# bayesian-optimization/BayesianOptimization

Measured on AMD Instinct MI355X. Metric: acquisition candidates/sec (suggest step: GP fit at fixed theta + posterior + acquisition + arg-best), higher is better.
Workload: dtype f64

## Files before the change

### bayesianoptimization_amd/_lib.py

```python
from __future__ import annotations

import ctypes as C
import os

import numpy as np

_HERE = os.path.dirname(os.path.abspath(__file__))
LIB_PATH = os.path.join(_HERE, "libgpbo.so")
DEBUG_LIB_PATH = os.path.join(_HERE, "libgpbo_dbg.so")

GPBO_OK = 0
ERR_INVALID, ERR_HIP, ERR_NOT_PD, ERR_STATE, ERR_UNSUPPORTED, ERR_COMM, ERR_PEER = -1, -2, -3, -4, -5, -6, -7
MAX_MODELS = 8
MAX_DIM = 64
MAX_SEEDS = 64
ABI_VERSION = 2

_c_double_p = C.POINTER(C.c_double)
_c_int64_p = C.POINTER(C.c_int64)
_c_int_p = C.POINTER(C.c_int)

SIGNATURES = {
    "gpbo_abi_version": (C.c_int, []),
    "gpbo_device_count": (C.c_int, [C.POINTER(C.c_int)]),
# ... 64 lines not shown
    "gpbo_group_fit_append": (C.c_int, [C.c_void_p, C.c_int, _c_double_p, C.c_int64, C.c_int, _c_double_p, C.c_int64,
                                        C.POINTER(C.c_int)]),
    "gpbo_group_lml_batch": (C.c_int, [C.c_void_p, C.c_int, _c_double_p, _c_double_p, C.c_int64, C.c_int, C.c_int, _c_double_p,
                                       C.c_int, C.c_double, C.c_int, _c_double_p, _c_double_p, C.POINTER(C.c_int),
                                       C.POINTER(C.c_int)]),
    "gpbo_group_set_candidates": (C.c_int, [C.c_void_p, _c_double_p, C.c_int64, C.c_int]),
    "gpbo_group_generate_candidates_mt19937": (C.c_int, [C.c_void_p, C.c_int64, C.c_int, _c_double_p, _c_double_p,
                                                         C.POINTER(C.c_uint32), C.POINTER(C.c_int)]),
    "gpbo_group_shard": (C.c_int, [C.c_void_p, C.c_int, _c_int64_p, _c_int64_p]),
    "gpbo_group_posterior": (C.c_int, [C.c_void_p, C.c_int, C.c_double, C.c_double, _c_double_p, _c_double_p]),
    "gpbo_group_acq_argbest": (C.c_int, [C.c_void_p, C.c_int, C.c_double, C.c_double, C.c_int, _c_double_p,
                                         _c_double_p, C.c_int, _c_int64_p, _c_double_p, _c_int64_p, _c_double_p,
                                         _c_double_p]),
    "gpbo_group_get_candidate_rows": (C.c_int, [C.c_void_p, _c_int64_p, C.c_int, _c_double_p]),
    "gpbo_polish_seeds": (C.c_int, [C.c_void_p, C.c_int, C.c_double, C.c_double, C.c_int, _c_double_p, _c_double_p, _c_double_p,
                                    _c_double_p, _c_double_p, C.c_int, C.c_int, _c_double_p, _c_double_p, C.c_int, _c_double_p,
                                    _c_double_p, C.POINTER(C.c_int), C.POINTER(C.c_int), C.POINTER(C.c_int), C.POINTER(C.c_int)]),
    "gpbo_evolve_mixed": (C.c_int, [C.c_void_p, C.c_int, C.c_double, C.c_double, C.c_double, C.c_double, C.c_int, _c_int_p,
                                    _c_int_p, _c_int_p, _c_double_p, _c_double_p, _c_double_p, C.c_int, C.c_int, C.c_int,
                                    C.POINTER(C.c_uint32), _c_int_p, _c_double_p, _c_double_p, _c_int_p, _c_int_p, _c_int_p]),
    "gpbo_mfma_f64_peak": (C.c_int, [C.c_void_p, C.c_int, _c_double_p]),
    "gpbo_mfma_f64_probe": (C.c_int, [C.c_void_p, C.c_int, C.c_int, C.c_int, _c_double_p]),
    "gpbo_hbm_copy_peak": (C.c_int, [C.c_void_p, C.c_int64, _c_double_p]),
}

DEBUG_SIGNATURES = {
    "gpbo_debug_minimize_box": (C.c_int, [C.c_void_p, C.c_void_p, _c_double_p, C.c_int, C.c_int, _c_double_p, _c_double_p, C.c_int,
                                          _c_double_p, _c_double_p, C.POINTER(C.c_int), C.POINTER(C.c_int), C.POINTER(C.c_int),
                                          C.POINTER(C.c_int)]),
    "gpbo_group_debug_create": (C.c_int, [C.c_int, C.POINTER(C.c_void_p)]),
    "gpbo_group_debug_run": (C.c_int, [C.c_void_p, C.c_int, C.c_int, C.c_int, C.c_int]),
    "gpbo_debug_cholesky": (C.c_int, [C.c_void_p, _c_double_p, C.c_int64, C.c_int, C.c_int, _c_double_p, _c_double_p,
                                      C.POINTER(C.c_int64), C.POINTER(C.c_double), C.POINTER(C.c_int)]),
    "gpbo_debug_latency_probe": (C.c_int, [C.c_void_p, C.POINTER(C.c_int64), C.c_int]),
    "gpbo_debug_select": (C.c_int, [C.c_void_p, C.c_void_p, C.c_int64, C.c_int, C.c_int, C.c_int, C.POINTER(C.c_int64), C.c_void_p,
                                    C.POINTER(C.c_int64), C.POINTER(C.c_float)]),
    "gpbo_debug_gemm": (C.c_int, [C.c_void_p, C.c_int, C.c_int, C.c_int, C.c_double, _c_double_p, _c_double_p,
                                  C.c_int, C.c_double, _c_double_p]),
    "gpbo_debug_gemm_bench": (C.c_int, [C.c_void_p, C.c_int, C.c_int, C.c_int, C.c_int, C.c_int, C.c_int, C.c_int,
                                        _c_double_p]),
    "gpbo_hybrid_probe": (C.c_int, [C.c_void_p, C.c_int, C.c_int, _c_double_p]),
    "gpbo_debug_fail_next_acq": (C.c_int, [C.c_void_p]),
    "gpbo_debug_evolve_eval": (C.c_int, [C.c_void_p, C.c_int, C.c_double, C.c_double, C.c_double, C.c_double, C.c_int, _c_int_p,
                                         _c_int_p, _c_int_p, _c_double_p, C.c_int, C.c_int, _c_double_p]),
    "gpbo_debug_evolve_walk": (C.c_int, [C.c_void_p, _c_double_p, _c_double_p, C.c_double, C.c_double, C.c_int, _c_int_p, _c_int_p,
                                         _c_int_p, _c_double_p, _c_double_p, _c_double_p, C.c_int, C.c_int, C.c_int, C.c_int,
                                         C.POINTER(C.c_uint32), _c_int_p, _c_double_p, _c_double_p, _c_int_p, _c_int_p, _c_int_p,
                                         _c_int_p]),
    "gpbo_debug_polish_eval": (C.c_int, [C.c_void_p, C.c_int, C.c_double, C.c_double, C.c_double, C.c_double, _c_double_p, C.c_int, C.c_int,
                                         C.c_int, _c_double_p]),
    "gpbo_debug_i8_pack_w": (C.c_int, [C.c_void_p, _c_double_p, C.c_int64, C.c_int64, C.c_void_p, _c_int_p, _c_double_p]),
    "gpbo_debug_i8_kstar_digits": (C.c_int, [C.c_void_p, C.c_int64, C.c_int64, C.c_int64, C.c_void_p, _c_double_p, _c_double_p]),
    "gpbo_debug_i8_gemm": (C.c_int, [C.c_void_p, C.c_void_p, _c_double_p, C.c_void_p, C.c_int64, C.c_int64, _c_double_p]),
}

_lib = None
_debug_lib = None


class GpboError(RuntimeError):
    """HIP / state / communicator failure reported by libgpbo."""


def _bind(path: str, signatures: dict):
    lib = C.CDLL(path)
    for name, (res, args) in signatures.items():
        fn = getattr(lib, name)
        fn.restype = res
        fn.argtypes = args
    if lib.gpbo_abi_version() != ABI_VERSION:
        raise ImportError(f"libgpbo ABI {lib.gpbo_abi_version()} != expected {ABI_VERSION}; rebuild")
    return lib


def load_library(path: str | None = None):
    global _lib
    if _lib is not None and path is None:
        return _lib
    explicit = path is not None
    path = path or LIB_PATH
    if not os.path.exists(path) and not explicit:
        try:
            from .build import build
            build(verbose=False)
        except Exception as e:
            raise ImportError(f"{path} not found and building it failed ({e}). There is no CPU fallback.") from e
    if not os.path.exists(path):
        raise ImportError(
            f"{path} not found: the HIP extension has not been built. Run "
            "`python -m bayesianoptimization_amd.build` (needs hipcc). There is no CPU fallback.")
    lib = _bind(path, SIGNATURES)
    if not explicit:
        _lib = lib
    return lib


def load_debug_library():
    global _debug_lib
    if _debug_lib is None:
        if not os.path.exists(DEBUG_LIB_PATH):
            try:
                from .build import build_debug
                build_debug(verbose=False)
            except Exception as e:
                raise ImportError(f"{DEBUG_LIB_PATH} not found and building it failed ({e})") from e
        _debug_lib = _bind(DEBUG_LIB_PATH, {**SIGNATURES, **DEBUG_SIGNATURES})
# ... 40 lines not shown
```

### bayesianoptimization_amd/csrc/i8_digits.h

```cpp
#pragma once

#include <cmath>
#include <cstdint>

#include "posterior_plan.h"

#if defined(__HIPCC__)
#define GPBO_HD __host__ __device__
#else
#define GPBO_HD
#endif

namespace gpbo {

static_assert((int64_t)I8_S * 128 * 128 * I8_NP_MAX < ((int64_t)1 << 31), "int32 level sums overflow at I8_NP_MAX");

template <int S>
GPBO_HD constexpr int64_t i8_offset() {
  int64_t o = 0;
  for (int t = 1; t < S; ++t) o = o * 256 + 128;
  return o;
}

GPBO_HD inline int64_t i8_round(double x) {
#if defined(__HIP_DEVICE_COMPILE__)
  return __double2ll_rn(x);
#else
  return (int64_t)std::nearbyint(x);
#endif
}

template <int S>
GPBO_HD inline int64_t i8_quantize(double x) {
  return i8_round(std::ldexp(x, 8 * S - 2)) + i8_offset<S>();
}

template <int S>
GPBO_HD inline uint32_t i8_digit_byte(int64_t Qo, int t) {
  return (uint32_t)((Qo >> (8 * (S - 1 - t))) & 255) ^ (t ? 128u : 0u);
}

GPBO_HD inline int i8_row_exponent(double maxabs) {
  int e = 0;
  (void)std::frexp(maxabs, &e);
  return maxabs > 0.0 ? e : 0;
}

template <int S>
GPBO_HD constexpr int64_t i8_frag_index(int64_t first_step, int64_t k, int plane, int item) {
  return ((first_step + (k >> 6)) * S + plane) * 64 + ((k >> 4) & 3) * 16 + item;
}
GPBO_HD constexpr int64_t i8_kd_block(int64_t cb, int64_t NP) { return cb * (NP / 64); }
GPBO_HD constexpr int64_t i8_wd_block(int64_t b) {
  const int64_t q = b >> 2, r = b & 3;
  return b + 2 * q * (q - 1) + r * q;
}

template <int S>
GPBO_HD inline double i8_combine(const int32_t* acc) {
  static_assert(S >= 5 && S <= 7, "groups of S - 4, 2 and 2 levels");
  double h = 0.0;
  for (int l = 0; l < S - 4; ++l) h = h * 256.0 + (double)acc[l];
  h *= 4294967296.0;
  const double m = (double)acc[S - 4] * 16777216.0 + (double)acc[S - 3] * 65536.0;
  const double lo = (double)acc[S - 2] * 256.0 + (double)acc[S - 1];
  const double s = h + m;
  const double bb = s - h;
  const double e = (h - (s - bb)) + (m - bb);
  return s + (e + lo);
}

template <int S>
GPBO_HD constexpr int i8_scale_exp(int e) {
  return e - 2 * (8 * S - 2) + 8 * (S - 1);
}

}
```

### bayesianoptimization_amd/csrc/posterior_i8.hip

```cpp
#include <algorithm>

#include "gpbo_internal.h"
#include "i8_digits.h"
#include "posterior_tile.h"

namespace gpbo {

typedef int v4i __attribute__((ext_vector_type(4)));

constexpr int I8_CANDS = 64;

__global__ __launch_bounds__(256) void wd_row_scale_kernel(const double* __restrict__ W, int* __restrict__ wexp,
                                                           double* __restrict__ wscale, int64_t N, int64_t NP) {
  const int64_t row = (int64_t)blockIdx.x * 4 + (threadIdx.x >> 6);
  const int lane = threadIdx.x & 63;
  if (row >= NP) return;
  double mx = 0.0;
  if (row < N)
    for (int64_t j = lane; j <= row; j += 64) mx = fmax(mx, fabs(W[row * NP + j]));
#pragma unroll
  for (int o = 32; o > 0; o >>= 1) mx = fmax(mx, __shfl_xor(mx, o));
  if (lane == 0) {
    const int e = i8_row_exponent(mx);
    wexp[row] = e;
// ... 199 lines not shown
  GPBO_HIP(ctx, hipSetDevice(ctx->device));
  Model m;
  m.N = N; m.NP = NP;
  auto done = [&](int code) {
    if (m.W) (void)hipFree(m.W);
    if (m.Wd) (void)hipFree(m.Wd);
    if (m.wscale) (void)hipFree(m.wscale);
    return code;
  };
  const size_t sq = (size_t)NP * NP * sizeof(double);
  if (hipMalloc((void**)&m.W, sq) != hipSuccess) return done(GPBO_ERR_HIP);
  if (hipMemcpy(m.W, W, sq, hipMemcpyHostToDevice) != hipSuccess) return done(GPBO_ERR_HIP);
  int rc = pack_wd(ctx, m);
  if (rc) return done(rc);
  if (hipStreamSynchronize(ctx->stream) != hipSuccess) return done(GPBO_ERR_HIP);
  const size_t wd_bytes = (size_t)i8_wd_block(NP / 16) * I8_S * 64 * sizeof(uint4);
  if (hipMemcpy(Wd_out, m.Wd, wd_bytes, hipMemcpyDeviceToHost) != hipSuccess) return done(GPBO_ERR_HIP);
  if (hipMemcpy(wscale_out, m.wscale, (size_t)NP * sizeof(double), hipMemcpyDeviceToHost) != hipSuccess) return done(GPBO_ERR_HIP);
  if (hipMemcpy(wexp_out, m.wscale + NP, (size_t)NP * sizeof(int), hipMemcpyDeviceToHost) != hipSuccess) return done(GPBO_ERR_HIP);
  return done(GPBO_OK);
}

int gpbo_debug_i8_gemm(gpbo_ctx* ctx, const void* Wd, const double* wscale, const void* Kd, int64_t NP, int64_t M, double* part_out) {
  if (!ctx) return GPBO_ERR_INVALID;
  if (!Wd || !wscale || !Kd || !part_out || !i8_debug_np_ok(NP) || M < I8_CANDS || M % I8_CANDS || M > (1 << 20))
    GPBO_FAIL(ctx, GPBO_ERR_INVALID, "debug_i8_gemm: bad arguments (NP a multiple of 64 in [64, 16384], M a multiple of 64)");
  GPBO_HIP(ctx, hipSetDevice(ctx->device));
  const int nchunks = (int)((NP + I8_ROWS - 1) / I8_ROWS);
  const size_t wd_bytes = (size_t)i8_wd_block(NP / 16) * I8_S * 64 * sizeof(uint4);
  const size_t kd_bytes = (size_t)M * NP * I8_S;
  const size_t part_bytes = (size_t)nchunks * M * sizeof(double);
  uint4 *dW = nullptr, *dK = nullptr;
  double *dS = nullptr, *dP = nullptr;
  auto done = [&](int code) {
    if (dW) (void)hipFree(dW);
    if (dK) (void)hipFree(dK);
    if (dS) (void)hipFree(dS);
    if (dP) (void)hipFree(dP);
    return code;
  };
  if (hipMalloc((void**)&dW, wd_bytes) != hipSuccess || hipMalloc((void**)&dK, kd_bytes) != hipSuccess ||
      hipMalloc((void**)&dS, (size_t)NP * sizeof(double)) != hipSuccess || hipMalloc((void**)&dP, part_bytes) != hipSuccess)
    return done(GPBO_ERR_HIP);
  if (hipMemcpy(dW, Wd, wd_bytes, hipMemcpyHostToDevice) != hipSuccess || hipMemcpy(dK, Kd, kd_bytes, hipMemcpyHostToDevice) != hipSuccess ||
      hipMemcpy(dS, wscale, (size_t)NP * sizeof(double), hipMemcpyHostToDevice) != hipSuccess ||
      hipMemset(dP, 0xff, part_bytes) != hipSuccess)
    return done(GPBO_ERR_HIP);
  const int rc = launch_i8_gemm(ctx, dW, dS, dK, dP, NP, M, nchunks, M, 0);
  if (rc) return done(rc);
  if (hipStreamSynchronize(ctx->stream) != hipSuccess) return done(GPBO_ERR_HIP);
  if (hipMemcpy(part_out, dP, part_bytes, hipMemcpyDeviceToHost) != hipSuccess) return done(GPBO_ERR_HIP);
  return done(GPBO_OK);
}
#endif
```

### bayesianoptimization_amd/csrc/posterior_kernel_v2.hip

```cpp
#include <type_traits>

#include "gpbo_internal.h"
#include "fit_bodies.h"
#include "i8_digits.h"
#include "posterior_tile.h"

namespace gpbo {

typedef double d4 __attribute__((ext_vector_type(4)));

constexpr int V2_CANDS = 64;
constexpr int V2_STRIDE = 64;

struct PostArgs2 {
  const double* Wp;
  const double* Xs;
  const double* alpha;
  const double* Xcs;
  double* part;
  double* mu_part;
  PostGrid g;
  const double* Kst;
  int64_t ldk;
  int64_t m0;
  int fuse_ends = 0;
  PostEnds ends = {};
};

template <int DP, int KERNEL, int GEN, int BK = POST_BK, int WAVES = 8>
__global__ __launch_bounds__(WAVES * 64, 4) void posterior_kernel_v2(PostArgs2 p) {
  static_assert(GEN == 1 || GEN == 2, "k* generated in the kernel or read from a slab");
  static_assert(BK == 16 || BK == 32, "stages of 16 or 32 train points");
  static_assert(WAVES == 8 || (WAVES == 16 && GEN == 1 && BK == 32), "the 16-wave form is the fused kernel with 32-point stages");
  constexpr int NT = WAVES * 64;
  constexpr int ROWS = WAVES * 32;
  constexpr int E = BK / WAVES;
  static_assert(GEN == 2 || E == 2 || E == 4, "the in-kernel generation computes train points in pairs: one or two pairs per thread and stage");
  constexpr int KP = BK / 8;
  extern __shared__ __attribute__((aligned(16))) double smem2[];
  double* Ks = smem2;
  double* Xl = smem2 + 2 * BK * V2_STRIDE;

  const int tid = threadIdx.x;
  const int wave = __builtin_amdgcn_readfirstlane(tid >> 6);
  const int lane = tid & 63;
  int r, ct;
  p.g.map(blockIdx.x, r, ct);
  const bool last = (r == p.g.nchunks - 1);
  const int NP = p.g.NP;
  const int k_end = min(NP, (r + 1) * ROWS);
  const int n_stages = k_end / BK;

  if constexpr (GEN != 2) {
    if (p.fuse_ends) {
      for (int e = tid; e < V2_CANDS * DP; e += NT) {
        const int cnd = e / DP, t = e - cnd * DP;
        const int64_t row = (int64_t)ct * V2_CANDS + cnd;
        double v = 0.0;
        if (row < p.ends.M && t < p.ends.d) v = p.ends.Xc[row * p.ends.d + t] / p.ends.ls[t];
        Xl[t * V2_CANDS + cnd] = v;
      }
    } else {
// ... 139 lines not shown
  for (; s <= last_stage; ++s) stage(s, std::integral_constant<int, 0>{});

  static_assert(2 * WAVES * V2_CANDS <= 2 * BK * V2_STRIDE, "the epilogue's exchange area aliases the stage tiles");
  double* red = Ks;
  double* mured = Ks + WAVES * V2_CANDS;
#pragma unroll
  for (int jt = 0; jt < 4; ++jt) {
    double v = 0.0;
#pragma unroll
    for (int rr = 0; rr < 4; ++rr) v = fma(acc[0][jt][rr], acc[0][jt][rr], v);
    if (!activeA) v = 0.0;
    double vb = 0.0;
#pragma unroll
    for (int rr = 0; rr < 4; ++rr) vb = fma(acc[1][jt][rr], acc[1][jt][rr], vb);
    if (activeB) v += vb;
    v += __shfl_xor(v, 16);
    v += __shfl_xor(v, 32);
    if (lane < 16) red[wave * V2_CANDS + jt * 16 + lane] = v;
  }
  mured[wave * V2_CANDS + lane] = mu_acc;
  __syncthreads();
  if (tid < V2_CANDS) {
    double v = 0.0;
#pragma unroll
    for (int w = 0; w < WAVES; ++w) v += red[w * V2_CANDS + tid];
    const int64_t m = p.m0 + (int64_t)ct * V2_CANDS + tid;
    if (GEN != 2 && p.fuse_ends) {
      double u = 0.0;
#pragma unroll
      for (int w = 0; w < WAVES; ++w) u += mured[w * V2_CANDS + tid];
      if (m < p.ends.M)
        posterior_finalize_elem(0.0 + v, 0.0 + u, p.ends.y_mean, p.ends.y_std, p.ends.mu + m, p.ends.sd + m, p.ends.negvar);
      return;
    }
    p.part[(int64_t)r * p.g.Mp + m] = v;
    if (GEN != 2 && last) {
      double u = 0.0;
#pragma unroll
      for (int w = 0; w < WAVES; ++w) u += mured[w * V2_CANDS + tid];
      p.mu_part[m] = u;
    }
  }
}

constexpr int GEN_CH = 64;
template <PostPath SLAB> struct slab_value { using type = double; };
template <> struct slab_value<PostPath::SlabF32> { using type = float; };
template <int DP, int KERNEL, PostPath SLAB>
__global__ __launch_bounds__(256) void kstar_gen_kernel(const double* __restrict__ Xs, const double* __restrict__ alpha,
                                                        const double* __restrict__ Xcs, void* __restrict__ slab,
                                                        int64_t ldk, int NP, double* __restrict__ mu_part,
                                                        int64_t Mp, int64_t m0) {
  static_assert(SLAB == PostPath::SlabF64 || SLAB == PostPath::SlabF32 || SLAB == PostPath::SlabI8, "a slab path");
  __shared__ __attribute__((aligned(16))) double xs[GEN_CH * DP];
  __shared__ double al[GEN_CH];
  const int64_t ml = (int64_t)blockIdx.x * 256 + threadIdx.x;
  const bool live = ml < ldk;
  const int k0 = blockIdx.y * POST_ROWS, k1 = min(NP, k0 + POST_ROWS);
  double xc[DP];
  {
    const double* xcp = Xcs + (m0 + (live ? ml : 0)) * DP;
#pragma unroll
    for (int t = 0; t < DP; t += 2) {
      const double2 v = *reinterpret_cast<const double2*>(xcp + t);
      xc[t] = v.x;
      xc[t + 1] = v.y;
    }
  }
  double mu = 0.0;
  auto pair = [&](int kk, double& ka, double& kb) {
    const double* xr = xs + kk * DP;
    double d2a = 0.0, d2b = 0.0;
#pragma unroll
    for (int t = 0; t < DP; ++t) {
      const double da = xc[t] - xr[t], db = xc[t] - xr[DP + t];
      d2a = fma(da, da, d2a);
      d2b = fma(db, db, d2b);
    }
    ka = gpbo_kernel_value<KERNEL>(d2a);
    kb = gpbo_kernel_value<KERNEL>(d2b);
  };
  auto mean = [&](int kk, double ka, double kb) {
    mu = fma(ka, al[kk], mu);
    mu = fma(kb, al[kk + 1], mu);
  };
  for (int kc = k0; kc < k1; kc += GEN_CH) {
    __syncthreads();
    {
      const double2* src = reinterpret_cast<const double2*>(Xs + (int64_t)kc * DP);
      double2* dst = reinterpret_cast<double2*>(xs);
      for (int e = threadIdx.x; e < GEN_CH * DP / 2; e += 256) dst[e] = src[e];
      if (threadIdx.x < GEN_CH) al[threadIdx.x] = alpha[kc + threadIdx.x];
    }
    __syncthreads();
    if (!live) continue;
    if constexpr (SLAB == PostPath::SlabI8) {
      constexpr int S = I8_S;
      uint4* Kd = static_cast<uint4*>(slab);
      const int64_t cb = i8_kd_block(ml >> 4, NP);
#pragma unroll 1
      for (int kg = 0; kg < GEN_CH; kg += 16) {
        uint32_t w[S][4] = {};
#pragma unroll
        for (int kk = kg; kk < kg + 16; kk += 2) {
          double ka, kb;
          pair(kk, ka, kb);
          mean(kk, ka, kb);
          const int64_t qa = i8_quantize<S>(ka), qb = i8_quantize<S>(kb);
          const int j = kk - kg;
#pragma unroll
          for (int t = 0; t < S; ++t) {
            w[t][j >> 2] |= (uint32_t)((qa >> (8 * (S - 1 - t))) & 255) << (8 * (j & 3));
            w[t][j >> 2] |= (uint32_t)((qb >> (8 * (S - 1 - t))) & 255) << (8 * ((j + 1) & 3));
          }
        }
        const int k = kc + kg;
        uint4* dst = Kd + i8_frag_index<S>(cb, k, 0, (int)(ml & 15));
#pragma unroll
        for (int t = 0; t < S; ++t) {
          const uint32_t x = t ? 0x80808080u : 0u;
          dst[t * 64] = make_uint4(w[t][0] ^ x, w[t][1] ^ x, w[t][2] ^ x, w[t][3] ^ x);
        }
      }
    } else {
      using T = typename slab_value<SLAB>::type;
      T* Kst = static_cast<T*>(slab);
#pragma unroll 2
      for (int kk = 0; kk < GEN_CH; kk += 2) {
        double ka, kb;
        pair(kk, ka, kb);
        const int k = kc + kk;
        Kst[(int64_t)k * ldk + ml] = (T)ka;
        Kst[(int64_t)(k + 1) * ldk + ml] = (T)kb;
        mean(kk, ka, kb);
      }
    }
  }
  if (live) mu_part[(int64_t)blockIdx.y * Mp + m0 + ml] = mu;
}

template <PostPath SLAB>
static int launch_gen(gpbo_ctx* ctx, Model& m, void* slab, int64_t ldk, int64_t Mp, int64_t m0, int nchunks) {
  return with_dp_kernel(ctx, m.DP, m.kernel, [&](auto dp, auto k) {
    kstar_gen_kernel<decltype(dp)::value, decltype(k)::value, SLAB><<<dim3((unsigned)((ldk + 255) / 256), (unsigned)nchunks), dim3(256), 0,
                                                                      ctx->stream>>>(m.Xs, m.alpha, ctx->Xcs, slab, ldk, (int)m.NP,
                                                                                     ctx->mu_part, Mp, m0);
    GPBO_HIP(ctx, hipGetLastError());
    return GPBO_OK;
  });
}

int launch_kstar_slab(gpbo_ctx* ctx, Model& m, double* Kst, int64_t ldk, int64_t Mp, int64_t m0, int nchunks) {
  return launch_gen<PostPath::SlabF64>(ctx, m, Kst, ldk, Mp, m0, nchunks);
}
int launch_kstar_slab_f32(gpbo_ctx* ctx, Model& m, float* Kst, int64_t ldk, int64_t Mp, int64_t m0, int nchunks) {
  return launch_gen<PostPath::SlabF32>(ctx, m, Kst, ldk, Mp, m0, nchunks);
}
int launch_kstar_digits(gpbo_ctx* ctx, Model& m, void* Kd, int64_t ldk, int64_t Mp, int64_t m0, int nchunks) {
  return launch_gen<PostPath::SlabI8>(ctx, m, Kd, ldk, Mp, m0, nchunks);
}

static PostArgs2 post_args(gpbo_ctx* ctx, const Model& m, int64_t Mp, int nchunks, int64_t ncands) {
  PostArgs2 a;
  a.Wp = m.Wp; a.Xs = m.Xs; a.alpha = m.alpha; a.Xcs = ctx->Xcs; a.part = ctx->part; a.mu_part = ctx->mu_part;
  a.g = {(int)m.NP, Mp, nchunks, (int)(ncands / V2_CANDS)};
  a.Kst = nullptr; a.ldk = 0; a.m0 = 0;
  return a;
}

int launch_slab_gemm_f64(gpbo_ctx* ctx, Model& m, const double* slab, int64_t ldk, int64_t m0, int64_t Mp, int part_chunks) {
  PostArgs2 a = post_args(ctx, m, Mp, part_chunks, ldk);
  a.Kst = slab; a.ldk = ldk; a.m0 = m0;
  const size_t lds = (size_t)(2 * 32 * V2_STRIDE) * sizeof(double);
  posterior_kernel_v2<4, 0, 2, 32><<<dim3((unsigned)a.g.blocks()), dim3(512), lds, ctx->stream>>>(a);
  GPBO_HIP(ctx, hipGetLastError());
  return GPBO_OK;
}

int launch_posterior_fused(gpbo_ctx* ctx, Model& m, int64_t Mp, const PostPlan& plan, const PostEnds& ends) {
  if (plan.fuse_ends && plan.part_chunks != 1) GPBO_FAIL(ctx, GPBO_ERR_STATE, "posterior: fused ends need one row chunk");
  PostArgs2 a = post_args(ctx, m, Mp, plan.part_chunks, Mp);
  const int64_t nblocks = a.g.blocks();
  if (nblocks > 0x7fffffffLL) GPBO_FAIL(ctx, GPBO_ERR_UNSUPPORTED, "posterior: grid too large; shard the candidates");
  if (plan.fuse_ends) { a.fuse_ends = 1; a.ends = ends; }
  const bool wide = plan.path == PostPath::Fused512;
  return with_dp_kernel(ctx, m.DP, m.kernel, [&](auto dp, auto k) {
    constexpr int DP = decltype(dp)::value, KERNEL = decltype(k)::value;
    if (wide) {
      const size_t lds = (size_t)(2 * 32 * V2_STRIDE + DP * V2_CANDS) * sizeof(double);
      posterior_kernel_v2<DP, KERNEL, 1, 32, 16><<<dim3((unsigned)nblocks), dim3(1024), lds, ctx->stream>>>(a);
// ... 56 lines not shown
```

### bayesianoptimization_amd/engine.py

```python
from __future__ import annotations

import contextlib
import ctypes as C
import json

import numpy as np

from . import _lib
from ._lib import dptr, iptr

RBF, MATERN25 = 0, 1
UCB, EI, POI = 0, 1, 2
F64, F32 = 0, 1

TIMING_NAMES = ("fit", "posterior_main", "posterior_finalize", "acq_argbest", "kmat", "cholesky", "trtri")


def advance_mt19937(random_state, n_words: int, lib=None):
    lib = lib or _lib.load_library()
    name, key, pos, has_gauss, cached = random_state.get_state(legacy=True)
    if name != "MT19937":
        raise TypeError("advance_mt19937 needs an MT19937 RandomState")
    n_words = int(n_words)
    avail = 624 - int(pos)
# ... 531 lines not shown
        first_nan, ms = C.c_int64(-1), C.c_float(0.0)
        self._check(self._lib.gpbo_debug_select(self._h, dptr(ys), ys.shape[0], int(k), int(variant), int(iters),
                                                idx.ctypes.data_as(C.POINTER(C.c_int64)), dptr(vals), C.byref(first_nan), C.byref(ms)))
        return idx, vals, int(first_nan.value), float(ms.value)

    def latency_probe(self, n=16):
        self._need_debug("gpbo_debug_latency_probe")
        out = np.zeros(32, dtype=np.int64)
        self._check(self._lib.gpbo_debug_latency_probe(self._h, out.ctypes.data_as(C.POINTER(C.c_int64)), int(n)))
        return out[:n]

    def debug_gemm(self, A, B, C_in=None, alpha=1.0, beta=0.0, b_trans=False):
        self._need_debug("gpbo_debug_gemm")
        A = np.ascontiguousarray(A, dtype=np.float64)
        B = np.ascontiguousarray(B, dtype=np.float64)
        m, k = A.shape
        n = B.shape[0] if b_trans else B.shape[1]
        Cm = np.zeros((m, n)) if C_in is None else np.ascontiguousarray(C_in, dtype=np.float64).copy()
        self._check(self._lib.gpbo_debug_gemm(self._h, m, n, k, float(alpha), dptr(A), dptr(B), int(b_trans),
                                              float(beta), dptr(Cm)))
        return Cm

    I8_S = 7

    @staticmethod
    def _i8_wd_bytes(NP: int) -> int:
        q = NP // 64
        return (NP // 16 + 2 * q * (q - 1)) * GpEngine.I8_S * 64 * 16

    def debug_i8_pack_w(self, W, N: int):
        self._need_debug("gpbo_debug_i8_pack_w")
        W = np.ascontiguousarray(W, dtype=np.float64)
        NP = W.shape[0]
        if W.ndim != 2 or W.shape[1] != NP or NP % 64 or not 64 <= NP <= 16384:
            raise ValueError("debug_i8_pack_w: W must be NP x NP, NP a multiple of 64 in [64, 16384]")
        Wd = np.empty(self._i8_wd_bytes(NP), dtype=np.int8)
        wexp = np.empty(NP, dtype=np.int32)
        wscale = np.empty(NP)
        self._check(self._lib.gpbo_debug_i8_pack_w(self._h, dptr(W), int(N), NP, Wd.ctypes.data_as(C.c_void_p),
                                                   wexp.ctypes.data_as(C.POINTER(C.c_int)), dptr(wscale)))
        return Wd, wexp, wscale

    def debug_i8_kstar_digits(self, NP: int, m0: int, ldk: int):
        self._need_debug("gpbo_debug_i8_kstar_digits")
        if NP % 64 or not 64 <= NP <= 16384 or ldk < 64:
            raise ValueError("debug_i8_kstar_digits: NP a multiple of 64 in [64, 16384], ldk >= 64")
        Kd = np.empty(int(ldk) * NP * self.I8_S, dtype=np.int8)
        kst = np.empty((NP, int(ldk)))
        mu_part = np.empty((2, (NP + 255) // 256, int(ldk)))
        self._check(self._lib.gpbo_debug_i8_kstar_digits(self._h, int(NP), int(m0), int(ldk), Kd.ctypes.data_as(C.c_void_p), dptr(kst),
                                                         dptr(mu_part)))
        return Kd, kst, mu_part

    def debug_i8_gemm(self, Wd, wscale, Kd, NP: int, M: int):
        self._need_debug("gpbo_debug_i8_gemm")
        Wd = np.ascontiguousarray(Wd, dtype=np.int8)
        Kd = np.ascontiguousarray(Kd, dtype=np.int8)
        wscale = np.ascontiguousarray(wscale, dtype=np.float64)
        if NP % 64 or not 64 <= NP <= 16384 or M % 64 or M < 64:
            raise ValueError("debug_i8_gemm: NP a multiple of 64 in [64, 16384], M a multiple of 64")
        if Wd.size != self._i8_wd_bytes(NP) or Kd.size != M * NP * self.I8_S or wscale.size != NP:
            raise ValueError("debug_i8_gemm: operand sizes do not match NP and M")
        part = np.empty(((NP + 127) // 128, M))
        self._check(self._lib.gpbo_debug_i8_gemm(self._h, Wd.ctypes.data_as(C.c_void_p), dptr(wscale), Kd.ctypes.data_as(C.c_void_p),
                                                 NP, M, dptr(part)))
        return part

    def gemm_bench(self, m, n, k, b_trans=True, a_trans=False, lower_only=False, iters=10) -> dict:
        self._need_debug("gpbo_debug_gemm_bench")
        out = np.zeros(2)
        self._check(self._lib.gpbo_debug_gemm_bench(self._h, int(m), int(n), int(k), int(b_trans), int(a_trans),
                                                    int(lower_only), int(iters), dptr(out)))
        return {"ms": float(out[0]), "tflops": float(out[1])}

    def mfma_f64_peak(self, iters=20000) -> float:
        out = C.c_double(0.0)
        self._check(self._lib.gpbo_mfma_f64_peak(self._h, int(iters), C.byref(out)))
        return out.value

    def mfma_f64_probe(self, iters=20000, waves_per_simd=1, mode=0) -> dict:
        out = np.zeros(4)
        self._check(self._lib.gpbo_mfma_f64_probe(self._h, int(iters), int(waves_per_simd), int(mode), dptr(out)))
        return {"tflops": out[0], "cycles_per_mfma": out[1], "shader_mhz": out[2], "ms": out[3]}

    def hybrid_probe(self, iters=2000, cfg=2) -> dict:
        self._need_debug("gpbo_hybrid_probe")
        out = np.zeros(3)
        self._check(self._lib.gpbo_hybrid_probe(self._h, int(iters), int(cfg), dptr(out)))
        return {"ms": out[0], "mfma_tflops": out[1], "valu_tflops": out[2]}

    def hbm_copy_peak(self, nbytes=1 << 30) -> float:
        out = C.c_double(0.0)
        self._check(self._lib.gpbo_hbm_copy_peak(self._h, int(nbytes), C.byref(out)))
        return out.value

    @staticmethod
    def comm_unique_id() -> bytes:
        lib = _lib.load_library()
        buf = C.create_string_buffer(128)
        rc = lib.gpbo_comm_unique_id(buf)
        if rc != _lib.GPBO_OK:
            _lib.raise_for_status(lib, None, rc)
        return buf.raw

    def comm_init(self, unique_id: bytes, world_size: int, rank: int):
        assert len(unique_id) == 128
# ... 278 lines not shown
```

### include/gpbo.h

```cpp
#ifndef GPBO_H
#define GPBO_H

#include <stdint.h>

#ifdef __cplusplus
extern "C" {
#endif

#define GPBO_ABI_VERSION 2

enum gpbo_status {
  GPBO_OK = 0,
  GPBO_ERR_INVALID = -1,
  GPBO_ERR_HIP = -2,
  GPBO_ERR_NOT_PD = -3,
  GPBO_ERR_STATE = -4,
  GPBO_ERR_UNSUPPORTED = -5,
  GPBO_ERR_COMM = -6,
  GPBO_ERR_PEER = -7
};

enum gpbo_kernel { GPBO_KERNEL_RBF = 0, GPBO_KERNEL_MATERN25 = 1 };
enum gpbo_acq { GPBO_ACQ_UCB = 0, GPBO_ACQ_EI = 1, GPBO_ACQ_POI = 2 };
enum gpbo_precision { GPBO_F64 = 0, GPBO_F32 = 1 };
// ... 107 lines not shown
                   const double* length_scale, int n_ls, double noise, int precision, int* info);
int gpbo_group_fit_append(gpbo_group* grp, int slot, const double* x_new, int64_t n_new, int d, const double* y_norm,
                          int64_t n_total, int* info);
int gpbo_group_lml_batch(gpbo_group* grp, int n_theta, const double* X, const double* y_norm, int64_t N, int d, int kernel,
                         const double* length_scales, int n_ls, double noise, int eval_gradient, double* lml, double* grad,
                         int* info, int* lane_device);
int gpbo_group_set_candidates(gpbo_group* grp, const double* Xc, int64_t M, int d);
int gpbo_group_shard(const gpbo_group* grp, int rank, int64_t* row_begin, int64_t* row_end);
int gpbo_group_generate_candidates_mt19937(gpbo_group* grp, int64_t M, int d, const double* lo, const double* hi,
                                           uint32_t* key, int* pos);
int gpbo_group_posterior(gpbo_group* grp, int slot, double y_mean, double y_std, double* mu, double* sd);
int gpbo_group_acq_argbest(gpbo_group* grp, int acq, double acq_param, double y_max, int n_constraints,
                           const double* lb, const double* ub, int k_seeds, int64_t* best_idx, double* best_val,
                           int64_t* seed_idx, double* seed_val, double* ys_out);
int gpbo_group_get_candidate_rows(gpbo_group* grp, const int64_t* idx, int n, double* out);

int gpbo_mfma_f64_peak(gpbo_ctx* ctx, int iters, double* tflops);
int gpbo_mfma_f64_probe(gpbo_ctx* ctx, int iters, int waves_per_simd, int mode, double* out);
int gpbo_hbm_copy_peak(gpbo_ctx* ctx, int64_t bytes, double* gbps);

#ifdef GPBO_DEBUG
typedef int (*gpbo_fg_callback)(const double* x, int n_live, int d, double* f, double* g, void* user);
int gpbo_debug_minimize_box(gpbo_fg_callback fg, void* user, const double* seeds, int n_seeds, int d, const double* box_lo,
                            const double* box_hi, int max_iter, double* x_out, double* f_out, int* status_out, int* n_rounds_out,
                            int* n_iter_out, int* n_eval_out);

int gpbo_debug_polish_eval(gpbo_ctx* ctx, int acq, double acq_param, double y_max, double y_mean, double y_std, const double* points,
                           int n, int d, int repeat, double* out);

int gpbo_debug_evolve_eval(gpbo_ctx* ctx, int acq, double acq_param, double y_max, double y_mean, double y_std, int n_groups,
                           const int* kind, const int* col0, const int* ncols, const double* points, int n, int D, double* out);
int gpbo_debug_evolve_walk(gpbo_ctx* ctx, const double* weights, const double* targets, double nan_below, double inf_above,
                           int n_groups, const int* kind, const int* col0, const int* ncols, const double* bounds_lo,
                           const double* bounds_hi, const double* init, int S, int D, int maxiter, int budget, unsigned* key,
                           int* pos, double* x_out, double* f_out, int* nit_out, int* nfev_out, int* success_out,
                           int* launches_out);

int gpbo_group_debug_create(int n_ranks, gpbo_group** out);
int gpbo_group_debug_run(gpbo_group* grp, int fail_rank, int fail_code, int hang_rank, int hang_ms);
int gpbo_debug_fail_next_acq(gpbo_ctx* ctx);
int gpbo_debug_cholesky(gpbo_ctx* ctx, const double* A, int64_t n, int variant, int iters, double* L_out, double* dinv_out,
                        long long* stamps_out, double* ms_out, int* info_out);
int gpbo_debug_gemm(gpbo_ctx* ctx, int m, int n, int k, double alpha, const double* A,
                    const double* B, int b_trans, double beta, double* C);
int gpbo_debug_gemm_bench(gpbo_ctx* ctx, int m, int n, int k, int b_trans, int a_trans, int lower_only, int iters,
                          double* out);
int gpbo_debug_select(gpbo_ctx* ctx, const double* ys, int64_t M, int k, int variant, int iters, int64_t* idx_out,
                      double* val_out, int64_t* first_nan_out, float* ms_out);
int gpbo_debug_latency_probe(gpbo_ctx* ctx, long long* out, int n);
int gpbo_hybrid_probe(gpbo_ctx* ctx, int iters, int cfg, double* out);
int gpbo_debug_i8_pack_w(gpbo_ctx* ctx, const double* W, int64_t N, int64_t NP, void* Wd_out, int* wexp_out, double* wscale_out);
int gpbo_debug_i8_kstar_digits(gpbo_ctx* ctx, int64_t NP, int64_t m0, int64_t ldk, void* Kd_out, double* kst_out, double* mu_part_out);
int gpbo_debug_i8_gemm(gpbo_ctx* ctx, const void* Wd, const double* wscale, const void* Kd, int64_t NP, int64_t M, double* part_out);
#endif

#ifdef __cplusplus
}
#endif
#endif
```

Before: 5.959 million.

## Double-buffer K* generation tiles and split int8 digits via byte permutes

The K* generation kernel now double-buffers the X/alpha chunk in shared memory and prefetches the next chunk into registers while computing the current one, so global loads overlap with kernel evaluation and one barrier per chunk is dropped. For the int8 slab path with small dimension, quantization into digit planes uses a magic-constant double trick plus v_perm byte shuffles on four values at once, replacing per-digit shifts and ORs. The change adds register pressure from the prefetch buffer and a second shared-memory buffer, which may lower occupancy. A debug entry point for testing the split is also added.

New measurement: 6.004 million, median of 6. No clear change (+0.8%).

```diff
diff --git a/bayesianoptimization_amd/_lib.py b/bayesianoptimization_amd/_lib.py
--- a/bayesianoptimization_amd/_lib.py
+++ b/bayesianoptimization_amd/_lib.py
@@ -140,6 +140,7 @@
     "gpbo_debug_i8_pack_w": (C.c_int, [C.c_void_p, _c_double_p, C.c_int64, C.c_int64, C.c_void_p, _c_int_p, _c_double_p]),
     "gpbo_debug_i8_kstar_digits": (C.c_int, [C.c_void_p, C.c_int64, C.c_int64, C.c_int64, C.c_void_p, _c_double_p, _c_double_p]),
     "gpbo_debug_i8_gemm": (C.c_int, [C.c_void_p, C.c_void_p, _c_double_p, C.c_void_p, C.c_int64, C.c_int64, _c_double_p]),
+    "gpbo_debug_i8_split": (C.c_int, [C.c_void_p, _c_double_p, C.c_int64, C.c_void_p]),
 }
 
 _lib = None
diff --git a/bayesianoptimization_amd/csrc/i8_digits.h b/bayesianoptimization_amd/csrc/i8_digits.h
--- a/bayesianoptimization_amd/csrc/i8_digits.h
+++ b/bayesianoptimization_amd/csrc/i8_digits.h
@@ -2,6 +2,7 @@
 
 #include <cmath>
 #include <cstdint>
+#include <cstring>
 
 #include "posterior_plan.h"
 
@@ -40,6 +41,66 @@
   return (uint32_t)((Qo >> (8 * (S - 1 - t))) & 255) ^ (t ? 128u : 0u);
 }
 
+
+GPBO_HD inline uint32_t i8_perm(uint32_t hi, uint32_t lo, uint32_t sel) {
+#if defined(__HIP_DEVICE_COMPILE__)
+  return __builtin_amdgcn_perm(hi, lo, sel);
+#else
+  const uint64_t v = ((uint64_t)hi << 32) | lo;
+  uint32_t r = 0;
+  for (int i = 0; i < 4; ++i) r |= (uint32_t)((v >> (8 * ((sel >> (8 * i)) & 7))) & 255) << (8 * i);
+  return r;
+#endif
+}
+
+GPBO_HD inline void i8_double_words(double x, uint32_t& lo, uint32_t& hi) {
+  uint64_t b;
+  std::memcpy(&b, &x, sizeof b);
+  lo = (uint32_t)b;
+  hi = (uint32_t)(b >> 32);
+}
+
+template <int S>
+GPBO_HD inline void i8_quantize_words(double k, uint32_t& lo, uint32_t& hi) {
+  static_assert(S >= 5 && S <= 7, "Q + OFF in two words, the upper one holding S - 4 planes");
+  constexpr double C = 6755399441055744.0;
+  constexpr double two32 = 4294967296.0;
+  constexpr double up_h = (double)((int64_t)1 << (8 * S - 34)), up_q = (double)((int64_t)1 << (8 * S - 2));
+  const double mh = k * up_h + C;
+  const double h = mh - C;
+  const double ml = std::fma(k, up_q, -(h * two32)) + C;
+  uint32_t h_lo, h_hi, l_lo, l_hi;
+  i8_double_words(mh, h_lo, h_hi);
+  i8_double_words(ml, l_lo, l_hi);
+  (void)h_hi;
+  const uint32_t q_hi = h_lo + (l_hi - 0x43380000u);
+  constexpr uint32_t off_lo = (uint32_t)i8_offset<S>(), off_hi = (uint32_t)(i8_offset<S>() >> 32);
+  lo = l_lo + off_lo;
+  hi = q_hi + off_hi + (lo < l_lo ? 1u : 0u);
+}
+
+template <int S>
+GPBO_HD inline void i8_split4(double k0, double k1, double k2, double k3, uint32_t (&w)[S]) {
+  uint32_t lo[4], hi[4];
+  i8_quantize_words<S>(k0, lo[0], hi[0]);
+  i8_quantize_words<S>(k1, lo[1], hi[1]);
+  i8_quantize_words<S>(k2, lo[2], hi[2]);
+  i8_quantize_words<S>(k3, lo[3], hi[3]);
+  constexpr uint32_t EVEN = 0x05010400u, ODD = 0x07030602u;
+  constexpr uint32_t LOW = 0x05040100u, HIGH = 0x07060302u;
+  constexpr uint32_t X = 0x80808080u;
+  const uint32_t l01e = i8_perm(lo[1], lo[0], EVEN), l23e = i8_perm(lo[3], lo[2], EVEN);
+  const uint32_t l01o = i8_perm(lo[1], lo[0], ODD), l23o = i8_perm(lo[3], lo[2], ODD);
+  w[S - 1] = i8_perm(l23e, l01e, LOW) ^ X;
+  w[S - 2] = i8_perm(l23e, l01e, HIGH) ^ X;
+  w[S - 3] = i8_perm(l23o, l01o, LOW) ^ X;
+  w[S - 4] = i8_perm(l23o, l01o, HIGH) ^ X;
+  const uint32_t h01e = i8_perm(hi[1], hi[0], EVEN), h23e = i8_perm(hi[3], hi[2], EVEN);
+  const uint32_t h01o = i8_perm(hi[1], hi[0], ODD), h23o = i8_perm(hi[3], hi[2], ODD);
+  const uint32_t hp[4] = {i8_perm(h23e, h01e, LOW), i8_perm(h23e, h01e, HIGH), i8_perm(h23o, h01o, LOW), i8_perm(h23o, h01o, HIGH)};
+  for (int b = 0; b < S - 4; ++b) w[S - 5 - b] = (S - 5 - b) ? hp[b] ^ X : hp[b];
+}
+
 GPBO_HD inline int i8_row_exponent(double maxabs) {
   int e = 0;
   (void)std::frexp(maxabs, &e);
diff --git a/bayesianoptimization_amd/csrc/posterior_i8.hip b/bayesianoptimization_amd/csrc/posterior_i8.hip
--- a/bayesianoptimization_amd/csrc/posterior_i8.hip
+++ b/bayesianoptimization_amd/csrc/posterior_i8.hip
@@ -275,4 +275,29 @@
   if (hipMemcpy(part_out, dP, part_bytes, hipMemcpyDeviceToHost) != hipSuccess) return done(GPBO_ERR_HIP);
   return done(GPBO_OK);
 }
+
+__global__ void i8_split_kernel(const double* __restrict__ k, int64_t n4, uint32_t* __restrict__ out) {
+  const int64_t i = (int64_t)blockIdx.x * blockDim.x + threadIdx.x;
+  if (i < n4) i8_split4<I8_S>(k[4 * i], k[4 * i + 1], k[4 * i + 2], k[4 * i + 3], *reinterpret_cast<uint32_t(*)[I8_S]>(out + i * I8_S));
+}
+
+int gpbo_debug_i8_split(gpbo_ctx* ctx, const double* k, int64_t n, void* out) {
+  if (!ctx) return GPBO_ERR_INVALID;
+  if (!k || !out || n < 16 || n % 16 || n > (1 << 26)) GPBO_FAIL(ctx, GPBO_ERR_INVALID, "debug_i8_split: bad arguments (n a multiple of 16, at most 2^26)");
+  GPBO_HIP(ctx, hipSetDevice(ctx->device));
+  const size_t in_bytes = (size_t)n * sizeof(double), out_bytes = (size_t)(n / 4) * I8_S * sizeof(uint32_t);
+  double* dk = nullptr;
+  uint32_t* dw = nullptr;
+  auto done = [&](int code) {
+    if (dk) (void)hipFree(dk);
+    if (dw) (void)hipFree(dw);
+    return code;
+  };
+  if (hipMalloc((void**)&dk, in_bytes) != hipSuccess || hipMalloc((void**)&dw, out_bytes) != hipSuccess) return done(GPBO_ERR_HIP);
+  if (hipMemcpy(dk, k, in_bytes, hipMemcpyHostToDevice) != hipSuccess) return done(GPBO_ERR_HIP);
+  i8_split_kernel<<<dim3((unsigned)((n / 4 + 255) / 256)), dim3(256), 0, ctx->stream>>>(dk, n / 4, dw);
+  if (hipGetLastError() != hipSuccess || hipStreamSynchronize(ctx->stream) != hipSuccess) return done(GPBO_ERR_HIP);
+  if (hipMemcpy(out, dw, out_bytes, hipMemcpyDeviceToHost) != hipSuccess) return done(GPBO_ERR_HIP);
+  return done(GPBO_OK);
+}
 #endif
diff --git a/bayesianoptimization_amd/csrc/posterior_kernel_v2.hip b/bayesianoptimization_amd/csrc/posterior_kernel_v2.hip
--- a/bayesianoptimization_amd/csrc/posterior_kernel_v2.hip
+++ b/bayesianoptimization_amd/csrc/posterior_kernel_v2.hip
@@ -8,6 +8,7 @@
 namespace gpbo {
 
 typedef double d4 __attribute__((ext_vector_type(4)));
+typedef double d2 __attribute__((ext_vector_type(2)));
 
 constexpr int V2_CANDS = 64;
 constexpr int V2_STRIDE = 64;
@@ -253,8 +254,8 @@
                                                         int64_t ldk, int NP, double* __restrict__ mu_part,
                                                         int64_t Mp, int64_t m0) {
   static_assert(SLAB == PostPath::SlabF64 || SLAB == PostPath::SlabF32 || SLAB == PostPath::SlabI8, "a slab path");
-  __shared__ __attribute__((aligned(16))) double xs[GEN_CH * DP];
-  __shared__ double al[GEN_CH];
+  __shared__ __attribute__((aligned(16))) double xs2[2][GEN_CH * DP];
+  __shared__ double al2[2][GEN_CH];
   const int64_t ml = (int64_t)blockIdx.x * 256 + threadIdx.x;
   const bool live = ml < ldk;
   const int k0 = blockIdx.y * POST_ROWS, k1 = min(NP, k0 + POST_ROWS);
@@ -269,6 +270,8 @@
     }
   }
   double mu = 0.0;
+  const double* xs = xs2[0];
+  const double* al = al2[0];
   auto pair = [&](int kk, double& ka, double& kb) {
     const double* xr = xs + kk * DP;
     double d2a = 0.0, d2b = 0.0;
@@ -285,58 +288,93 @@
     mu = fma(ka, al[kk], mu);
     mu = fma(kb, al[kk + 1], mu);
   };
-  for (int kc = k0; kc < k1; kc += GEN_CH) {
+  constexpr bool AHEAD = !(SLAB == PostPath::SlabI8 && DP > 32);
+  constexpr int NX2 = GEN_CH * DP / 2;
+  constexpr int NX = (NX2 + 255) / 256;
+  const bool holds_x = NX2 % 256 == 0 || threadIdx.x < NX2 % 256, holds_a = threadIdx.x < GEN_CH;
+  d2 px[NX];
+  double pa = 0.0;
+#define GPBO_GEN_FETCH(kc_)                                                                              \
+  {                                                                                                      \
+    const d2* src = reinterpret_cast<const d2*>(Xs + (int64_t)(kc_) * DP) + threadIdx.x;                 \
+    _Pragma("unroll") for (int i = 0; i < NX; ++i) if (i + 1 < NX || holds_x) px[i] = src[i * 256];      \
+    if (holds_a) pa = alpha[(kc_) + threadIdx.x];                                                        \
+  }
+#define GPBO_GEN_LAND(buf_)                                                                              \
+  {                                                                                                      \
+    d2* dst = reinterpret_cast<d2*>(xs2[buf_]) + threadIdx.x;                                            \
+    _Pragma("unroll") for (int i = 0; i < NX; ++i) if (i + 1 < NX || holds_x) dst[i * 256] = px[i];      \
+    if (holds_a) al2[buf_][threadIdx.x] = pa;                                                            \
+  }
+  GPBO_GEN_FETCH(k0)
+  GPBO_GEN_LAND(0)
+  int buf = 0;
+  for (int kc = k0; kc < k1; kc += GEN_CH, buf ^= 1) {
+    const bool more = kc + GEN_CH < k1;
+    if (more) GPBO_GEN_FETCH(kc + GEN_CH)
+    if constexpr (AHEAD) __builtin_amdgcn_sched_barrier(0);
     __syncthreads();
-    {
-      const double2* src = reinterpret_cast<const double2*>(Xs + (int64_t)kc * DP);
-      double2* dst = reinterpret_cast<double2*>(xs);
-      for (int e = threadIdx.x; e < GEN_CH * DP / 2; e += 256) dst[e] = src[e];
-      if (threadIdx.x < GEN_CH) al[threadIdx.x] = alpha[kc + threadIdx.x];
-    }
-    __syncthreads();
-    if (!live) continue;
-    if constexpr (SLAB == PostPath::SlabI8) {
-      constexpr int S = I8_S;
-      uint4* Kd = static_cast<uint4*>(slab);
-      const int64_t cb = i8_kd_block(ml >> 4, NP);
+    if constexpr (!AHEAD) {
+      if (more) GPBO_GEN_LAND(buf ^ 1)
+    }
+    xs = xs2[buf];
+    al = al2[buf];
+    if (live) {
+      if constexpr (SLAB == PostPath::SlabI8) {
+        constexpr int S = I8_S;
+        uint4* Kd = static_cast<uint4*>(slab);
+        const int64_t cb = i8_kd_block(ml >> 4, NP);
 #pragma unroll 1
-      for (int kg = 0; kg < GEN_CH; kg += 16) {
-        uint32_t w[S][4] = {};
-#pragma unroll
-        for (int kk = kg; kk < kg + 16; kk += 2) {
+        for (int kg = 0; kg < GEN_CH; kg += 16) {
+          uint32_t w[4][S] = {};
+          if constexpr (DP <= 32) {
+#pragma unroll
+            for (int kk = kg; kk < kg + 16; kk += 4) {
+              double ka, kb, kc2, kd;
+              pair(kk, ka, kb);
+              mean(kk, ka, kb);
+              pair(kk + 2, kc2, kd);
+              mean(kk + 2, kc2, kd);
+              i8_split4<S>(ka, kb, kc2, kd, w[(kk - kg) >> 2]);
+            }
+          } else {
+#pragma unroll
+            for (int kk = kg; kk < kg + 16; kk += 2) {
+              double ka, kb;
+              pair(kk, ka, kb);
+              mean(kk, ka, kb);
+              const int64_t qa = i8_quantize<S>(ka), qb = i8_quantize<S>(kb);
+              const int j = kk - kg;
+#pragma unroll
+              for (int t = 0; t < S; ++t)
+                w[j >> 2][t] |= i8_digit_byte<S>(qa, t) << (8 * (j & 3)) | i8_digit_byte<S>(qb, t) << (8 * ((j + 1) & 3));
+            }
+          }
+          const int k = kc + kg;
+          uint4* dst = Kd + i8_frag_index<S>(cb, k, 0, (int)(ml & 15));
+#pragma unroll
+          for (int t = 0; t < S; ++t) dst[t * 64] = make_uint4(w[0][t], w[1][t], w[2][t], w[3][t]);
+        }
+      } else {
+        using T = typename slab_value<SLAB>::type;
+        T* Kst = static_cast<T*>(slab);
+#pragma unroll 2
+        for (int kk = 0; kk < GEN_CH; kk += 2) {
           double ka, kb;
           pair(kk, ka, kb);
+          const int k = kc + kk;
+          Kst[(int64_t)k * ldk + ml] = (T)ka;
+          Kst[(int64_t)(k + 1) * ldk + ml] = (T)kb;
           mean(kk, ka, kb);
-          const int64_t qa = i8_quantize<S>(ka), qb = i8_quantize<S>(kb);
-          const int j = kk - kg;
-#pragma unroll
-          for (int t = 0; t < S; ++t) {
-            w[t][j >> 2] |= (uint32_t)((qa >> (8 * (S - 1 - t))) & 255) << (8 * (j & 3));
-            w[t][j >> 2] |= (uint32_t)((qb >> (8 * (S - 1 - t))) & 255) << (8 * ((j + 1) & 3));
-          }
         }
-        const int k = kc + kg;
-        uint4* dst = Kd + i8_frag_index<S>(cb, k, 0, (int)(ml & 15));
-#pragma unroll
-        for (int t = 0; t < S; ++t) {
-          const uint32_t x = t ? 0x80808080u : 0u;
-          dst[t * 64] = make_uint4(w[t][0] ^ x, w[t][1] ^ x, w[t][2] ^ x, w[t][3] ^ x);
-        }
-      }
-    } else {
-      using T = typename slab_value<SLAB>::type;
-      T* Kst = static_cast<T*>(slab);
-#pragma unroll 2
-      for (int kk = 0; kk < GEN_CH; kk += 2) {
-        double ka, kb;
-        pair(kk, ka, kb);
-        const int k = kc + kk;
-        Kst[(int64_t)k * ldk + ml] = (T)ka;
-        Kst[(int64_t)(k + 1) * ldk + ml] = (T)kb;
-        mean(kk, ka, kb);
-      }
-    }
-  }
+      }
+    }
+    if constexpr (AHEAD) {
+      if (more) GPBO_GEN_LAND(buf ^ 1)
+    }
+  }
+#undef GPBO_GEN_FETCH
+#undef GPBO_GEN_LAND
   if (live) mu_part[(int64_t)blockIdx.y * Mp + m0 + ml] = mu;
 }
 
diff --git a/bayesianoptimization_amd/engine.py b/bayesianoptimization_amd/engine.py
--- a/bayesianoptimization_amd/engine.py
+++ b/bayesianoptimization_amd/engine.py
@@ -607,6 +607,15 @@
                                                          dptr(mu_part)))
         return Kd, kst, mu_part
 
+    def debug_i8_split(self, k):
+        self._need_debug("gpbo_debug_i8_split")
+        k = np.ascontiguousarray(k, dtype=np.float64).ravel()
+        if k.size < 16 or k.size % 16:
+            raise ValueError("debug_i8_split: a multiple of 16 values")
+        out = np.empty((k.size // 4, self.I8_S), dtype=np.uint32)
+        self._check(self._lib.gpbo_debug_i8_split(self._h, dptr(k), k.size, out.ctypes.data_as(C.c_void_p)))
+        return out
+
     def debug_i8_gemm(self, Wd, wscale, Kd, NP: int, M: int):
         self._need_debug("gpbo_debug_i8_gemm")
         Wd = np.ascontiguousarray(Wd, dtype=np.int8)
diff --git a/include/gpbo.h b/include/gpbo.h
--- a/include/gpbo.h
+++ b/include/gpbo.h
@@ -183,6 +183,7 @@
 int gpbo_debug_i8_pack_w(gpbo_ctx* ctx, const double* W, int64_t N, int64_t NP, void* Wd_out, int* wexp_out, double* wscale_out);
 int gpbo_debug_i8_kstar_digits(gpbo_ctx* ctx, int64_t NP, int64_t m0, int64_t ldk, void* Kd_out, double* kst_out, double* mu_part_out);
 int gpbo_debug_i8_gemm(gpbo_ctx* ctx, const void* Wd, const double* wscale, const void* Kd, int64_t NP, int64_t M, double* part_out);
+int gpbo_debug_i8_split(gpbo_ctx* ctx, const double* k, int64_t n, void* out);
 #endif
 
 #ifdef __cplusplus
```
